# SKSKSK94/Distributed_SAC

Measured on AMD Instinct MI355X. Metric: learner grad-steps/sec (aggregate over GPUs), MT10-MTSAC, higher is better.
Workload: dtype bf16; 1 GPU; global_batch=1280, seq_len=1, parallelism=dp1, batch_per_gpu=1280, update=full SAC step: TD target + critic/actor/alpha fwd+bwd+fusedAdam + Polyak, hipgraph=True, launch_mode=graph, graph_chunk=1

## Files before the change

distributed_sac_amd/algo/sac.py:

```python

from __future__ import annotations

from typing import Dict, Optional

import torch
import torch.nn as nn

from ..config import SACConfig
from ..models import Actor, Critic, LLActor, LLCritic
from ..ops import functional as Fops
from ..ops.flat import FlatParams, FusedAdam, flat_polyak_


class SACEngine:

    def __init__(self, cfg: SACConfig, device: torch.device | str = "cpu",
                 precision: Optional[str] = None):
        import os as _os
        self.precision = (precision or
                          _os.environ.get("DSAC_PRECISION", "fp32"))
        self.cfg = cfg
        self.variant = cfg.variant
        self.device = torch.device(device)
        self.gamma = cfg.gamma
# ... 132 lines not shown
            device=self.device)
        off = self.actor_group.adopt_grad_arena(self._aa_arena, 0)
        self.alpha_group.adopt_grad_arena(self._aa_arena, off)
        self._init_bf16_mirrors()
        self.hard_copy_targets()

    def _init_bf16_mirrors(self) -> None:
        self._bf16 = (self.precision == "bf16"
                      and self.device.type == "cuda")
        if not self._bf16:
            return
        dev = self.device
        self._loss_ws = torch.zeros(256, device=dev)
        self._aloss_ws = torch.zeros(256, device=dev)
        self._dla_ws = torch.zeros(2048, device=dev)
        self._rng_ctr = torch.tensor(
            [int(torch.initial_seed()) & 0x7FFFFFFF],
            dtype=torch.int64, device=dev)
        self._critic_bf16 = torch.empty(self.critic_group.numel,
                                        dtype=torch.bfloat16, device=dev)
        self._target_bf16 = torch.empty(self.target_group.numel,
                                        dtype=torch.bfloat16, device=dev)
        self._actor_bf16 = torch.empty(self.actor_group.numel,
                                       dtype=torch.bfloat16, device=dev)
        self._twin_local_bf16 = self._stack_views(self.critic_group,
                                                  self._critic_bf16,
                                                  self._critic_layer_pairs())
        self._twin_target_bf16 = self._stack_views(
            self.target_group, self._target_bf16,
            self._critic_layer_pairs(target=True))
# ... 286 lines not shown
            self.ddp.allreduce_grad_(self._aa_arena)
        return self._manual_seg3()

    @property
    def _use_chain(self) -> bool:
        import os as _os
        return _os.environ.get("DSAC_CHAIN", "1") == "1"

    @property
    def _use_krng(self) -> bool:
        import os as _os
        return (getattr(self, "_bf16", False)
                and getattr(self, "_rng_ctr", None) is not None
                and _os.environ.get("DSAC_KRNG", "1") == "1")

    def _adam_prolog_all(self) -> bool:
        from ..ops import native
        opts = [self.critic_optimizer, self.actor_optimizer,
                self.log_alpha_optimizer]
        ctx = getattr(self, "context_encoder_optimizer", None)
        if ctx is not None:
            opts.append(ctx)
        if any(o._dev_state is None for o in opts):
            return False
        b1, b2 = opts[0].betas
        if any(o.betas != (b1, b2) or o.eps != opts[0].eps for o in opts):
            return False
        native().adam_prolog_many(
            [o._dev_state for o in opts], [o.lr for o in opts], b1, b2,
            self._rng_ctr if self._use_krng else None)
# ... 62 lines not shown
            mu, lsr, eps, float(self.actor.k),
            self._rng_ctr if krng else None)
        na, nlp = a_cat[:B], lp_cat[:B]

        if chain:
            yt, _ = self._chain_fwd(next_states, na,
                                    self._twin_target_bf16,
                                    self._twin_target[1], G=2,
                                    save_acts=False,
                                    wps=self._twin_target_fp)
            q1_t, q2_t = yt[0], yt[1]
        else:
            xt = torch.cat([next_states, na], dim=-1)
            q1_t, q2_t, _ = self._twin_fwd_manual(
                xt, self._twin_target_bf16, self._twin_target[1])
        y = ext.td_target_mt(rewards, dones, q1_t, q2_t, nlp, states,
                             la_det, T, self.gamma, self.reward_scale)

        if chain:
            yq, acts_c = self._chain_fwd(states, actions,
                                         self._twin_local_bf16,
                                         self._twin_local[1], G=2,
                                         wps=self._twin_local_fp)
            q1, q2 = yq[0], yq[1]
        else:
            x = torch.cat([states, actions], dim=-1)
            q1, q2, acts_c = self._twin_fwd_manual(
                x, self._twin_local_bf16, self._twin_local[1])
        closs = ext.critic_loss_fwd(q1, q2, y, states, la_det, T,
                                    int(use_w), self._loss_ws)[0]
        dy = ext.critic_loss_bwd2(q1, q2, y, states, la_det, closs, T,
                                  int(use_w))
        wsg = [w.grad for w in self._twin_local[0]]
        bsg = [b.grad for b in self._twin_local[1]]
        fg_c = self.critic_group.flat_grad
        arena_c, S_c, ch_c = self._dw_arena("critic",
                                            self.critic_group.numel, B)
        if chain:
            nl_c = len(self._twin_local_bf16)
            empty_h = states.new_empty(0, dtype=torch.bfloat16)
            youts = [acts_c[i + 1] for i in range(nl_c - 1)] + [empty_h]
            aflags = [1] * (nl_c - 1) + [0]
            dys = ext.mlp_chain_dx_bf16(dy, list(self._twin_local_wt),
                                        youts, acts_c[0].shape[-1],
                                        aflags, 2, 1, -1,
                                        list(self._twin_local_dxp))
            base_c = fg_c.data_ptr()
            ext.dwdb_grouped_arena(
                list(dys), [acts_c[i] for i in range(nl_c)], arena_c,
                [(w.data_ptr() - base_c) // 4 for w in wsg],
                [(b.data_ptr() - base_c) // 4 for b in bsg],
                2, S_c, ch_c)
        else:
            self._mlp_bwd_arena(ext, dy, acts_c, self._twin_local_bf16,
                                wsg, bsg, fg_c, arena_c, S_c, ch_c, G=2)
        ext.reduce_arena(arena_c, fg_c, S_c)
        self._dp_st = {
            "states": states, "sa": a_cat[B:], "lp": lp_cat[B:],
            "lsr": lsr, "ls_cat": ls_cat, "eps": eps, "tanh_u": tanh_u,
            "acts_a": acts_a, "ws_f32": ws_f32, "bs_f32": bs_f32,
            "la_det": la_det, "closs": closs, "B": B,
        }

    @torch.no_grad()
    def _manual_seg2(self):
        from ..ops import native
        ext = native()
        st = self._dp_st
        st["prolog"] = self._adam_prolog_all()
        self.critic_optimizer.step(pre_prologed=st["prolog"])

        states, sa, lp = st["states"], st["sa"], st["lp"]
        B = st["B"]
        T = self.num_tasks
        use_w = self.use_weighted_loss
        la_det = st["la_det"]
        ls = st["ls_cat"][B:]
        nl_a = len(self._actor_ws_bf16)
        nl_c = len(self._twin_local_bf16)
        acts_a = st["acts_a"]

        if self._use_chain:
            ext.pack_weights_frag(
                list(self._twin_local_bf16) * 2,
                list(self._twin_local_fp) + list(self._twin_local_dxp),
                [2] * (2 * nl_c), [0] * nl_c + [1] * nl_c)
            ya, acts_f = self._chain_fwd(states, sa, self._twin_local_bf16,
                                         self._twin_local[1], G=2,
                                         wps=self._twin_local_fp)
            aq1, aq2 = ya[0], ya[1]
        else:
            xa = torch.cat([states, sa], dim=-1)
            aq1, aq2, acts_f = self._twin_fwd_manual(
                xa, self._twin_local_bf16, self._twin_local[1])
        al = ext.actor_alpha_loss_fwd(aq1, aq2, lp, ls, states,
                                      la_det, T, int(use_w), self.H_bar_f,
                                      self.alpha_group.flat_grad,
                                      self._aloss_ws)
        daq, dlp = ext.actor_alpha_loss_bwd2(
            aq1, aq2, lp, states, la_det, al, self.alpha_group.flat_grad,
            T, int(use_w), self.H_bar_f, self._dla_ws)
        if self._use_chain:
            empty_h = states.new_empty(0, dtype=torch.bfloat16)
            youts_f = [acts_f[i + 1] for i in range(nl_c - 1)] + [empty_h]
            outs = ext.mlp_chain_dx_bf16(
                daq, list(self._twin_local_wt), youts_f,
                acts_f[0].shape[-1], [1] * (nl_c - 1) + [0], 2, 0,
                states.shape[1], list(self._twin_local_dxp))
            dx0 = outs[-1]
            dsa = dx0
        else:
            dy = daq
            for i in range(nl_c - 1, 0, -1):
                act = 1 if i < nl_c - 1 else 0
                yout = acts_f[i + 1] if i < nl_c - 1 else acts_f[i]
                dy = ext.linear_bwd_dx_bf16(dy, self._twin_local_bf16[i],
# ... 27 lines not shown
                [(b.data_ptr() - base_a) // 4 for b in bag],
                1, S_a, ch_a)
        else:
            dy = dhead
            for i in range(nl_a - 1, -1, -1):
                act = 1 if i < nl_a - 1 else 0
                yout = (acts_a[i + 1][B:] if i < nl_a - 1
                        else acts_a[i][B:])
                ext.linear_bwd_dwdb_arena(
                    dy, acts_a[i][B:], yout, act, 1, arena_a,
                    (wag[i].data_ptr() - base_a) // 4,
                    (bag[i].data_ptr() - base_a) // 4, S_a, ch_a, 0)
                if i > 0:
                    dy = ext.linear_bwd_dx_bf16(dy, self._actor_ws_bf16[i],
                                                yout, act, 1, 1)
        ext.reduce_arena(arena_a, fg_a, S_a)
        st["al"] = al

    @torch.no_grad()
    def _manual_seg3(self):
        st = self._dp_st
        FusedAdam.step_many([self.actor_optimizer,
                             self.log_alpha_optimizer],
                            rng_bump=(None if st.get("prolog")
                                      else (self._rng_ctr if self._use_krng
                                            else None)),
                            pre_prologed=bool(st.get("prolog")))
        flat_polyak_(self.target_group, self.critic_group, self.tau,
                     mirror=getattr(self, "_target_bf16", None))
        closs, al = st["closs"], st["al"]
        return {
            "critic_loss": closs[6],
            "actor_loss": al[0],
            "alpha_loss": al[2],
            "entropy": al[3],
        }

    def _update_tensors_fused(self, batch):
        from ..ops import native
        states = batch["states"]
        actions = batch["actions"]
        rewards = batch["rewards"]
        next_states = batch["next_states"]
        dones = batch["dones"]
# ... 192 lines not shown
```

distributed_sac_amd/ops/_hip/dsac_kernels.hip:

```cpp

#include <hip/hip_runtime.h>
#include <torch/extension.h>
#include <ATen/hip/HIPContext.h>
#include <c10/hip/HIPStream.h>

#include <cmath>
#include <vector>

using f32x4 = __attribute__((__vector_size__(4 * sizeof(float)))) float;

static constexpr int BM = 64;
static constexpr int BN = 64;
static constexpr int BK = 32;
static constexpr int PAD_K = BK + 2;
static constexpr int PAD_N = 80;

#define CHECK_IN(t) TORCH_CHECK((t).is_cuda() && (t).scalar_type() == torch::kFloat32, \
                                #t " must be a fp32 HIP tensor")

static inline hipStream_t cur_stream() {
  return c10::hip::getCurrentHIPStream().stream();
}

__global__ __launch_bounds__(256) void k_linear_act_fwd(
// ... 383 lines not shown
    const float mask = (raw >= -20.f && raw <= 2.f) ? 1.f : 0.f;
    dlsr[idx] = mask * (du * e * s - g);
  }
}

__global__ __launch_bounds__(256) void k_td_target(
    const float* __restrict__ r, const float* __restrict__ d,
    const float* __restrict__ q1, const float* __restrict__ q2,
    const float* __restrict__ lp, const float* __restrict__ alpha,
    float* __restrict__ y, int n, float gamma, float rs) {
  const int i = blockIdx.x * blockDim.x + threadIdx.x;
  if (i >= n) return;
  y[i] = rs * r[i] + gamma * (1.f - d[i]) * (fminf(q1[i], q2[i]) - alpha[i] * lp[i]);
}

__global__ __launch_bounds__(256) void k_td_target_mt(
    const float* __restrict__ r, const float* __restrict__ d,
    const float* __restrict__ q1, const float* __restrict__ q2,
    const float* __restrict__ lp, const float* __restrict__ onehot,
    const float* __restrict__ log_alpha, float* __restrict__ y,
    int n, int T, int oh_stride, float gamma, float rs) {
  const int i = blockIdx.x * blockDim.x + threadIdx.x;
  if (i >= n) return;
  int t_i = 0;
  if (T > 1) {
    float best = -1e30f;
    for (int t = 0; t < T; ++t) {
      const float v = onehot[(long)i * oh_stride + t];
      if (v > best) { best = v; t_i = t; }
    }
  }
  const float alpha = __expf(log_alpha[t_i]);
  y[i] = rs * r[i] + gamma * (1.f - d[i]) * (fminf(q1[i], q2[i]) - alpha * lp[i]);
}


__device__ __forceinline__ int task_of_row(const float* __restrict__ onehot,
                                           long i, int oh_stride, int T) {
  if (T <= 1) return 0;
  int t_i = 0;
  float best = -1e30f;
  for (int t = 0; t < T; ++t) {
    const float v = onehot[i * oh_stride + t];
    if (v > best) { best = v; t_i = t; }
  }
  return t_i;
}

// ... 556 lines not shown
  m[i] = mi;
  v[i] = vi;
  const float pn = p[i] - st[1] * mi / (sqrtf(vi) * st[2] + eps);
  p[i] = pn;
  if (mr != nullptr) mr[i] = f32_bf16_rne_d(pn);
}

__global__ __launch_bounds__(256) void k_polyak(
    float* __restrict__ t, const float* __restrict__ s, long n, float tau,
    unsigned short* __restrict__ mir) {
  const long i = (long)blockIdx.x * blockDim.x + threadIdx.x;
  if (i >= n) return;
  const float tn = (1.f - tau) * t[i] + tau * s[i];
  t[i] = tn;
  if (mir != nullptr) mir[i] = f32_bf16_rne_d(tn);
}


static torch::Tensor linear_act_fwd_g(torch::Tensor x, torch::Tensor w,
                                      torch::Tensor b, long act, long G) {
  CHECK_IN(x); CHECK_IN(w); CHECK_IN(b);
  auto xc = x.contiguous(); auto wc = w.contiguous(); auto bc = b.contiguous();
  const bool per_group_x = xc.dim() == 3;
  const long M = per_group_x ? xc.size(1) : xc.size(0);
  const long K = xc.size(-1);
  const long N = wc.numel() / (G * K);
  TORCH_CHECK(wc.numel() == G * N * K && bc.numel() == G * N,
              "grouped weight shape mismatch");
  const long xgs = per_group_x ? M * K : 0;
  auto y = G == 1 ? torch::empty({M, N}, xc.options())
// ... 382 lines not shown
    ws_p = ws->data_ptr<float>();
  }
  hipLaunchKernelGGL(k_actor_alpha_loss_bwd2,
                     dim3(ws_p ? nblk : nblk + 1),
                     dim3(256),
                     ws_p ? 0 : (size_t)T * 256 * sizeof(float),
                     cur_stream(), aq1.data_ptr<float>(),
                     aq2.data_ptr<float>(), lp.data_ptr<float>(), oh,
                     log_alpha.data_ptr<float>(), saved.data_ptr<float>(),
                     (unsigned short*)daq.data_ptr(), dlp.data_ptr<float>(),
                     dla_out.data_ptr<float>(), ws_p, (int)B, (int)T,
                     (int)oh_stride, (int)use_w, (float)H_bar);
  return {daq, dlp};
}

static torch::Tensor squashed_gaussian_bwd2(
    torch::Tensor ga, torch::Tensor gl, torch::Tensor lsr, torch::Tensor ls,
    torch::Tensor eps, torch::Tensor tanh_u, double k) {
  CHECK_IN(ga);
  auto gac = ga.contiguous(); auto glc = gl.contiguous();
  const bool lsr_ok = lsr.dim() == 2 && lsr.stride(1) == 1;
  auto lsrc = lsr_ok ? lsr : lsr.contiguous();
  auto lsc = ls.contiguous();
  auto ec = eps.contiguous(); auto tc = tanh_u.contiguous();
  const int ga_twin = (gac.dim() == 3 && gac.size(0) == 2) ? 1 : 0;
  const long B = ga_twin ? gac.size(1) : gac.size(0);
  const long A = ga_twin ? gac.size(2) : gac.size(1);
  const long lsr_ld = lsr_ok ? lsr.stride(0) : A;
  auto dhead = torch::empty({B, 2 * A},
                            gac.options().dtype(torch::kBFloat16));
// ... 15 lines not shown
  const double bc1 = 1.0 - std::pow(b1, (double)step);
  const double bc2 = 1.0 - std::pow(b2, (double)step);
  const float step_size = (float)(lr / bc1);
  const float inv_sqrt_bc2 = (float)(1.0 / std::sqrt(bc2));
  hipLaunchKernelGGL(k_adam, dim3((n + 255) / 256), dim3(256), 0,
                     cur_stream(), p.data_ptr<float>(), g.data_ptr<float>(),
                     m.data_ptr<float>(), v.data_ptr<float>(), n,
                     (float)b1, (float)b2, step_size, inv_sqrt_bc2,
                     (float)eps);
}

static void adam_step_dev_(torch::Tensor p, torch::Tensor g, torch::Tensor m,
                           torch::Tensor v, torch::Tensor state, double lr,
                           double b1, double b2, double eps,
                           c10::optional<torch::Tensor> mir_opt,
                           long skip_prolog = 0) {
  CHECK_IN(p); CHECK_IN(state);
  TORCH_CHECK(state.numel() >= 3, "state = {step, step_size, inv_sqrt_bc2}");
  const long n = p.numel();
  unsigned short* mp = nullptr;
  if (mir_opt.has_value() && mir_opt->defined() && mir_opt->numel() > 0) {
    TORCH_CHECK(mir_opt->numel() == n
                && mir_opt->scalar_type() == torch::kBFloat16);
    mp = (unsigned short*)mir_opt->data_ptr();
  }
  if (!skip_prolog)
    hipLaunchKernelGGL(k_adam_prolog, dim3(1), dim3(1), 0, cur_stream(),
                       state.data_ptr<float>(), (float)lr, (float)b1,
                       (float)b2);
  hipLaunchKernelGGL(k_adam_dev, dim3((n + 255) / 256), dim3(256), 0,
                     cur_stream(), p.data_ptr<float>(), g.data_ptr<float>(),
                     m.data_ptr<float>(), v.data_ptr<float>(),
                     state.data_ptr<float>(), n, (float)b1, (float)b2,
                     (float)eps, mp);
}

static void adam_prolog_many(std::vector<torch::Tensor> states,
                             std::vector<double> lrs, double b1, double b2,
                             c10::optional<torch::Tensor> rng) {
  const size_t G = states.size();
  TORCH_CHECK(G >= 1 && G <= 4 && lrs.size() == G, "1..4 states");
  float* S[4] = {nullptr, nullptr, nullptr, nullptr};
  double L[4] = {0, 0, 0, 0};
  for (size_t g = 0; g < G; ++g) {
// ... 5 lines not shown
      ? (long long*)rng->data_ptr<long>() : nullptr;
  hipLaunchKernelGGL(k_adam_prolog_many, dim3(1), dim3(4), 0, cur_stream(),
                     rng_p, S[0], S[1], S[2], S[3], (float)L[0],
                     (float)L[1], (float)L[2], (float)L[3], (float)b1,
                     (float)b2);
}

static void adam_step_multi_(std::vector<torch::Tensor> ps,
                             std::vector<torch::Tensor> gs,
                             std::vector<torch::Tensor> ms,
                             std::vector<torch::Tensor> vs,
                             std::vector<torch::Tensor> states,
                             std::vector<double> lrs, double b1, double b2,
                             double eps, std::vector<torch::Tensor> mirs,
                             c10::optional<torch::Tensor> rng = c10::nullopt,
                             long skip_prolog = 0) {
  const size_t G = ps.size();
  TORCH_CHECK(G >= 1 && G <= 3, "1..3 groups");
  float* P[3] = {nullptr, nullptr, nullptr};
  const float* Gr[3] = {nullptr, nullptr, nullptr};
  float* M[3] = {nullptr, nullptr, nullptr};
  float* V[3] = {nullptr, nullptr, nullptr};
  float* St[3] = {nullptr, nullptr, nullptr};
  long N[3] = {0, 0, 0};
  double LR[3] = {0, 0, 0};
  unsigned short* MR[3] = {nullptr, nullptr, nullptr};
  long total = 0;
  for (size_t g = 0; g < G; ++g) {
    CHECK_IN(ps[g]);
    P[g] = ps[g].data_ptr<float>();
    Gr[g] = gs[g].data_ptr<float>();
// ... 3 lines not shown
    N[g] = ps[g].numel();
    LR[g] = lrs[g];
    if (g < mirs.size() && mirs[g].defined() && mirs[g].numel() > 0) {
      TORCH_CHECK(mirs[g].numel() == N[g]
                  && mirs[g].scalar_type() == torch::kBFloat16);
      MR[g] = (unsigned short*)mirs[g].data_ptr();
    }
    total += N[g];
  }
  long long* rng_p = (rng.has_value() && rng->numel() > 0)
      ? (long long*)rng->data_ptr<long>() : nullptr;
  if (!skip_prolog)
    hipLaunchKernelGGL(k_adam_prolog3, dim3(1), dim3(3), 0, cur_stream(),
                       rng_p, St[0], St[1], St[2], (float)LR[0],
                       (float)LR[1], (float)LR[2], (float)b1, (float)b2);
  hipLaunchKernelGGL(k_adam_multi, dim3((total + 255) / 256), dim3(256), 0,
                     cur_stream(),
                     P[0], Gr[0], M[0], V[0], St[0], N[0],
                     P[1], Gr[1], M[1], V[1], St[1], N[1],
                     P[2], Gr[2], M[2], V[2], St[2], N[2],
                     (float)b1, (float)b2, (float)eps, MR[0], MR[1], MR[2]);
}

static void polyak_(torch::Tensor t, torch::Tensor s, double tau,
                    c10::optional<torch::Tensor> mir_opt) {
  CHECK_IN(t);
  const long n = t.numel();
  TORCH_CHECK(s.numel() == n, "polyak buffers must match");
  unsigned short* mp = nullptr;
  if (mir_opt.has_value() && mir_opt->defined() && mir_opt->numel() > 0) {
// ... 44 lines not shown
          pybind11::arg("aq1"), pybind11::arg("aq2"),
          pybind11::arg("lp"), pybind11::arg("ls"),
          pybind11::arg("states"), pybind11::arg("log_alpha"),
          pybind11::arg("T"), pybind11::arg("use_w"),
          pybind11::arg("H_bar"),
          pybind11::arg("dla") = pybind11::none(),
          pybind11::arg("ws") = pybind11::none());
  mod.def("actor_alpha_loss_bwd", &actor_alpha_loss_bwd);
  mod.def("critic_loss_bwd2", &critic_loss_bwd2);
  mod.def("actor_alpha_loss_bwd2", &actor_alpha_loss_bwd2,
          pybind11::arg("aq1"), pybind11::arg("aq2"), pybind11::arg("lp"),
          pybind11::arg("states"), pybind11::arg("log_alpha"),
          pybind11::arg("saved"), pybind11::arg("dla_out"),
          pybind11::arg("T"), pybind11::arg("use_w"), pybind11::arg("H_bar"),
          pybind11::arg("ws") = pybind11::none());
  mod.def("squashed_gaussian_bwd2", &squashed_gaussian_bwd2);
  mod.def("adam_step_", &adam_step_);
  mod.def("adam_step_dev_", &adam_step_dev_,
          pybind11::arg("p"), pybind11::arg("g"), pybind11::arg("m"),
          pybind11::arg("v"), pybind11::arg("state"), pybind11::arg("lr"),
          pybind11::arg("b1"), pybind11::arg("b2"), pybind11::arg("eps"),
          pybind11::arg("mir") = pybind11::none(),
          pybind11::arg("skip_prolog") = 0);
  mod.def("adam_step_multi_", &adam_step_multi_,
          pybind11::arg("ps"), pybind11::arg("gs"), pybind11::arg("ms"),
          pybind11::arg("vs"), pybind11::arg("states"), pybind11::arg("lrs"),
          pybind11::arg("b1"), pybind11::arg("b2"), pybind11::arg("eps"),
          pybind11::arg("mirs") = std::vector<torch::Tensor>(),
          pybind11::arg("rng") = pybind11::none(),
          pybind11::arg("skip_prolog") = 0);
  mod.def("adam_prolog_many", &adam_prolog_many,
          pybind11::arg("states"), pybind11::arg("lrs"),
          pybind11::arg("b1"), pybind11::arg("b2"),
          pybind11::arg("rng") = pybind11::none());
  mod.def("polyak_", &polyak_,
          pybind11::arg("t"), pybind11::arg("s"), pybind11::arg("tau"),
          pybind11::arg("mir") = pybind11::none());
}
```

distributed_sac_amd/ops/flat.py:

```python

from __future__ import annotations

import math
from typing import Dict, Iterable, List, Optional

import torch
import torch.nn as nn

from . import has_native, native, native_enabled


def _flatten_into(params: List[torch.Tensor]) -> torch.Tensor:
    numel = sum(p.numel() for p in params)
    if numel == 0:
        return torch.empty(0)
    flat = torch.empty(numel, dtype=torch.float32, device=params[0].device)
    off = 0
    for p in params:
        n = p.numel()
        flat[off:off + n].copy_(p.detach().reshape(-1))
        off += n
    return flat


# ... 86 lines not shown
        if self._dev_state is not None:
            return int(self._dev_state[0].item())
        return self._step_count

    @step_count.setter
    def step_count(self, v: int) -> None:
        self._step_count = int(v)
        if self._dev_state is not None:
            with torch.no_grad():
                self._dev_state[0] = float(v)

    def zero_grad(self) -> None:
        self.group.zero_grad()

    @torch.no_grad()
    def step(self, pre_prologed: bool = False) -> None:
        p, g = self.group.flat_data, self.group.flat_grad
        m, v = self.exp_avg, self.exp_avg_sq
        b1, b2 = self.betas
        if self._dev_state is not None:
            native().adam_step_dev_(p, g, m, v, self._dev_state,
                                    self.lr, b1, b2, self.eps,
                                    self.bf16_mirror,
                                    1 if pre_prologed else 0)
            return
        self._step_count += 1
        bc1 = 1 - b1 ** self._step_count
        bc2 = 1 - b2 ** self._step_count
        m.mul_(b1).add_(g, alpha=1 - b1)
        v.mul_(b2).addcmul_(g, g, value=1 - b2)
        denom = (v.sqrt() / math.sqrt(bc2)).add_(self.eps)
        p.addcdiv_(m, denom, value=-self.lr / bc1)

    @staticmethod
    @torch.no_grad()
    def step_many(opts: List["FusedAdam"], rng_bump=None,
                  pre_prologed: bool = False) -> None:
        live = [o for o in opts if o is not None]
        if (1 <= len(live) <= 3
                and all(o._dev_state is not None for o in live)
                and all(o.betas == live[0].betas and o.eps == live[0].eps
                        for o in live)):
            native().adam_step_multi_(
                [o.group.flat_data for o in live],
                [o.group.flat_grad for o in live],
                [o.exp_avg for o in live],
                [o.exp_avg_sq for o in live],
                [o._dev_state for o in live],
                [o.lr for o in live],
                live[0].betas[0], live[0].betas[1], live[0].eps,
                [o.bf16_mirror if o.bf16_mirror is not None
                 else torch.Tensor() for o in live],
                rng_bump, 1 if pre_prologed else 0)
            return
        for o in live:
            o.step()


    def state_dict(self) -> Dict:
        state = {}
        for i, (p, off) in enumerate(zip(self.ref_params, self._ref_offsets)):
            n = p.numel()
            state[i] = {
                "step": torch.tensor(float(self.step_count)),
                "exp_avg": self.exp_avg[off:off + n].view_as(p.data).clone(),
                "exp_avg_sq": self.exp_avg_sq[off:off + n].view_as(p.data).clone(),
            }
        group = {
            "lr": self.lr, "betas": self.betas, "eps": self.eps,
            "weight_decay": 0, "amsgrad": False, "maximize": False,
            "foreach": None, "capturable": False, "differentiable": False,
# ... 31 lines not shown
```

Before: 3244 grad_steps/s.

## Fuse SAC step tail: TD+critic loss, actor/alpha loss, arena reduce into Adam, Polyak

Merges the TD-target, critic loss forward and critic loss backward into one kernel, using a last-block-done atomic for the cross-block reduction. It also merges the actor/alpha loss forward and backward into one kernel. On single-GPU runs, the per-slice gradient-arena reduction is folded into the Adam step kernels and the Polyak target update is folded into the actor/alpha Adam launch. Together these cut several small kernel launches per step, at the cost of more complex kernels with grid-wide atomics and redundant per-block weight-sum scans.

Result: faster. 3444 grad_steps/s, median of 6 (+6.1%).

```diff
diff --git a/distributed_sac_amd/algo/sac.py b/distributed_sac_amd/algo/sac.py
--- a/distributed_sac_amd/algo/sac.py
+++ b/distributed_sac_amd/algo/sac.py
@@ -170,6 +170,7 @@
         self._loss_ws = torch.zeros(256, device=dev)
         self._aloss_ws = torch.zeros(256, device=dev)
         self._dla_ws = torch.zeros(2048, device=dev)
+        self._aafb_ws = torch.zeros(1 + 32 * 4 + 32 * 32, device=dev)
         self._rng_ctr = torch.tensor(
             [int(torch.initial_seed()) & 0x7FFFFFFF],
             dtype=torch.int64, device=dev)
@@ -486,6 +487,11 @@
                 and getattr(self, "_rng_ctr", None) is not None
                 and _os.environ.get("DSAC_KRNG", "1") == "1")
 
+    @property
+    def _fuse_tail(self) -> bool:
+        import os as _os
+        return _os.environ.get("DSAC_FUSE_TAIL", "1") == "1"
+
     def _adam_prolog_all(self) -> bool:
         from ..ops import native
         opts = [self.critic_optimizer, self.actor_optimizer,
@@ -578,8 +584,11 @@
             xt = torch.cat([next_states, na], dim=-1)
             q1_t, q2_t, _ = self._twin_fwd_manual(
                 xt, self._twin_target_bf16, self._twin_target[1])
-        y = ext.td_target_mt(rewards, dones, q1_t, q2_t, nlp, states,
-                             la_det, T, self.gamma, self.reward_scale)
+        fuse = self._fuse_tail
+        fuse_loss = fuse and B <= 8192
+        if not fuse_loss:
+            y = ext.td_target_mt(rewards, dones, q1_t, q2_t, nlp, states,
+                                 la_det, T, self.gamma, self.reward_scale)
 
         if chain:
             yq, acts_c = self._chain_fwd(states, actions,
@@ -591,10 +600,15 @@
             x = torch.cat([states, actions], dim=-1)
             q1, q2, acts_c = self._twin_fwd_manual(
                 x, self._twin_local_bf16, self._twin_local[1])
-        closs = ext.critic_loss_fwd(q1, q2, y, states, la_det, T,
-                                    int(use_w), self._loss_ws)[0]
-        dy = ext.critic_loss_bwd2(q1, q2, y, states, la_det, closs, T,
-                                  int(use_w))
+        if fuse_loss:
+            closs, dy = ext.critic_td_loss(
+                rewards, dones, q1_t, q2_t, nlp, q1, q2, states, la_det, T,
+                int(use_w), self.gamma, self.reward_scale, self._loss_ws)
+        else:
+            closs = ext.critic_loss_fwd(q1, q2, y, states, la_det, T,
+                                        int(use_w), self._loss_ws)[0]
+            dy = ext.critic_loss_bwd2(q1, q2, y, states, la_det, closs, T,
+                                      int(use_w))
         wsg = [w.grad for w in self._twin_local[0]]
         bsg = [b.grad for b in self._twin_local[1]]
         fg_c = self.critic_group.flat_grad
@@ -618,8 +632,11 @@
         else:
             self._mlp_bwd_arena(ext, dy, acts_c, self._twin_local_bf16,
                                 wsg, bsg, fg_c, arena_c, S_c, ch_c, G=2)
-        ext.reduce_arena(arena_c, fg_c, S_c)
+        fold_c = fuse and self.ddp is None
+        if not fold_c:
+            ext.reduce_arena(arena_c, fg_c, S_c)
         self._dp_st = {
+            "fuse": fuse, "arena_c": (arena_c, S_c) if fold_c else None,
             "states": states, "sa": a_cat[B:], "lp": lp_cat[B:],
             "lsr": lsr, "ls_cat": ls_cat, "eps": eps, "tanh_u": tanh_u,
             "acts_a": acts_a, "ws_f32": ws_f32, "bs_f32": bs_f32,
@@ -632,7 +649,8 @@
         ext = native()
         st = self._dp_st
         st["prolog"] = self._adam_prolog_all()
-        self.critic_optimizer.step(pre_prologed=st["prolog"])
+        self.critic_optimizer.step(pre_prologed=st["prolog"],
+                                   arena=st["arena_c"])
 
         states, sa, lp = st["states"], st["sa"], st["lp"]
         B = st["B"]
@@ -657,13 +675,22 @@
             xa = torch.cat([states, sa], dim=-1)
             aq1, aq2, acts_f = self._twin_fwd_manual(
                 xa, self._twin_local_bf16, self._twin_local[1])
-        al = ext.actor_alpha_loss_fwd(aq1, aq2, lp, ls, states,
-                                      la_det, T, int(use_w), self.H_bar_f,
-                                      self.alpha_group.flat_grad,
-                                      self._aloss_ws)
-        daq, dlp = ext.actor_alpha_loss_bwd2(
-            aq1, aq2, lp, states, la_det, al, self.alpha_group.flat_grad,
-            T, int(use_w), self.H_bar_f, self._dla_ws)
+        fuse = st["fuse"]
+        if fuse and B <= 8192:
+            al, daq, dlp = ext.actor_alpha_loss_fwd_bwd(
+                aq1, aq2, lp, ls, states, la_det,
+                self.alpha_group.flat_grad, T, int(use_w), self.H_bar_f,
+                self._aafb_ws, st["closs"][2:3] if use_w else None)
+        else:
+            al = ext.actor_alpha_loss_fwd(aq1, aq2, lp, ls, states,
+                                          la_det, T, int(use_w),
+                                          self.H_bar_f,
+                                          self.alpha_group.flat_grad,
+                                          self._aloss_ws)
+            daq, dlp = ext.actor_alpha_loss_bwd2(
+                aq1, aq2, lp, states, la_det, al,
+                self.alpha_group.flat_grad, T, int(use_w), self.H_bar_f,
+                self._dla_ws)
         if self._use_chain:
             empty_h = states.new_empty(0, dtype=torch.bfloat16)
             youts_f = [acts_f[i + 1] for i in range(nl_c - 1)] + [empty_h]
@@ -721,20 +748,28 @@
                 if i > 0:
                     dy = ext.linear_bwd_dx_bf16(dy, self._actor_ws_bf16[i],
                                                 yout, act, 1, 1)
-        ext.reduce_arena(arena_a, fg_a, S_a)
+        fold_a = fuse and self.ddp is None
+        if not fold_a:
+            ext.reduce_arena(arena_a, fg_a, S_a)
+        st["arena_a"] = (arena_a, S_a) if fold_a else None
         st["al"] = al
 
     @torch.no_grad()
     def _manual_seg3(self):
         st = self._dp_st
+        polyak = (self.target_group, self.critic_group, self.tau,
+                  getattr(self, "_target_bf16", None))
+        fuse = bool(st.get("fuse"))
         FusedAdam.step_many([self.actor_optimizer,
                              self.log_alpha_optimizer],
                             rng_bump=(None if st.get("prolog")
                                       else (self._rng_ctr if self._use_krng
                                             else None)),
-                            pre_prologed=bool(st.get("prolog")))
-        flat_polyak_(self.target_group, self.critic_group, self.tau,
-                     mirror=getattr(self, "_target_bf16", None))
+                            pre_prologed=bool(st.get("prolog")),
+                            arena0=st.get("arena_a"),
+                            polyak=polyak if fuse else None)
+        if not fuse:
+            flat_polyak_(*polyak)
         closs, al = st["closs"], st["al"]
         return {
             "critic_loss": closs[6],
diff --git a/distributed_sac_amd/ops/_hip/dsac_kernels.hip b/distributed_sac_amd/ops/_hip/dsac_kernels.hip
--- a/distributed_sac_amd/ops/_hip/dsac_kernels.hip
+++ b/distributed_sac_amd/ops/_hip/dsac_kernels.hip
@@ -421,6 +421,15 @@
   y[i] = rs * r[i] + gamma * (1.f - d[i]) * (fminf(q1[i], q2[i]) - alpha[i] * lp[i]);
 }
 
+__device__ __forceinline__ float td_target_value(float rs, float r,
+                                                 float gamma, float d,
+                                                 float qmin, float alpha,
+                                                 float lp) {
+#pragma clang fp contract(off)
+  const float x = __builtin_fmaf(-alpha, lp, qmin);
+  return rs * r + gamma * (1.f - d) * x;
+}
+
 __global__ __launch_bounds__(256) void k_td_target_mt(
     const float* __restrict__ r, const float* __restrict__ d,
     const float* __restrict__ q1, const float* __restrict__ q2,
@@ -438,7 +447,8 @@
     }
   }
   const float alpha = __expf(log_alpha[t_i]);
-  y[i] = rs * r[i] + gamma * (1.f - d[i]) * (fminf(q1[i], q2[i]) - alpha * lp[i]);
+  y[i] = td_target_value(rs, r[i], gamma, d[i], fminf(q1[i], q2[i]), alpha,
+                         lp[i]);
 }
 
 
@@ -1025,6 +1035,362 @@
   const float tn = (1.f - tau) * t[i] + tau * s[i];
   t[i] = tn;
   if (mir != nullptr) mir[i] = f32_bf16_rne_d(tn);
+}
+
+
+struct __attribute__((packed, aligned(4))) OneHot4 { float v[4]; };
+struct __attribute__((packed, aligned(4))) OneHot2 { float v[2]; };
+
+__device__ __forceinline__ float batch_weight_sum(
+    const float* __restrict__ smw, const float* __restrict__ onehot,
+    float (*wpart)[4], int B, int T, int oh_stride, int nblk, int& own_t) {
+  const int tid = threadIdx.x, wid = tid >> 6, lane = tid & 63;
+  constexpr int KR = 8;
+  for (int b0 = 0; b0 < nblk; b0 += KR) {
+    float best[KR];
+    int ti[KR];
+    long row[KR];
+#pragma unroll
+    for (int k = 0; k < KR; ++k) {
+      const int i = (b0 + k) * 256 + tid;
+      row[k] = (long)(i < B ? i : B - 1);
+      best[k] = -1e30f;
+      ti[k] = 0;
+    }
+    if (T > 1) {
+      int t = 0;
+#pragma unroll 2
+      for (; t + 4 <= T; t += 4) {
+#pragma unroll
+        for (int k = 0; k < KR; ++k) {
+          const OneHot4 q = *reinterpret_cast<const OneHot4*>(
+              onehot + row[k] * oh_stride + t);
+#pragma unroll
+          for (int c = 0; c < 4; ++c)
+            if (q.v[c] > best[k]) { best[k] = q.v[c]; ti[k] = t + c; }
+        }
+      }
+      if (t + 2 <= T) {
+#pragma unroll
+        for (int k = 0; k < KR; ++k) {
+          const OneHot2 q = *reinterpret_cast<const OneHot2*>(
+              onehot + row[k] * oh_stride + t);
+#pragma unroll
+          for (int c = 0; c < 2; ++c)
+            if (q.v[c] > best[k]) { best[k] = q.v[c]; ti[k] = t + c; }
+        }
+        t += 2;
+      }
+      if (t < T) {
+#pragma unroll
+        for (int k = 0; k < KR; ++k) {
+          const float v = onehot[row[k] * oh_stride + t];
+          if (v > best[k]) { best[k] = v; ti[k] = t; }
+        }
+      }
+    }
+    float w[KR];
+#pragma unroll
+    for (int k = 0; k < KR; ++k) {
+      const int i = (b0 + k) * 256 + tid;
+      w[k] = i < B ? smw[ti[k]] : 0.f;
+      if (b0 + k == (int)blockIdx.x) own_t = ti[k];
+    }
+#pragma unroll
+    for (int off = 32; off > 0; off >>= 1) {
+#pragma unroll
+      for (int k = 0; k < KR; ++k) w[k] += __shfl_xor(w[k], off, 64);
+    }
+#pragma unroll
+    for (int k = 0; k < KR; ++k)
+      if (lane == 0 && b0 + k < nblk) wpart[b0 + k][wid] = w[k];
+  }
+  __syncthreads();
+  float r = 0.f;
+  for (int b = 0; b < nblk; ++b)
+    r += wpart[b][0] + wpart[b][1] + wpart[b][2] + wpart[b][3];
+  return r;
+}
+
+__global__ __launch_bounds__(256) void k_critic_td_loss(
+    const float* __restrict__ r, const float* __restrict__ d,
+    const float* __restrict__ q1t, const float* __restrict__ q2t,
+    const float* __restrict__ nlp, const float* __restrict__ q1,
+    const float* __restrict__ q2, const float* __restrict__ onehot,
+    const float* __restrict__ log_alpha, float* __restrict__ out,
+    float* __restrict__ ws, unsigned short* __restrict__ dq,
+    int B, int T, int oh_stride, int use_w, float gamma, float rs) {
+  __shared__ float part[3][4];
+  __shared__ float smw[32];
+  __shared__ float wpart[32][4];
+  __shared__ float s_fin[32 * 3];
+  __shared__ int s_last;
+  const int tid = threadIdx.x;
+  const int i = blockIdx.x * 256 + tid;
+  const long ic = i < B ? i : B - 1;
+  const float rv = r[ic], dv = d[ic], q1tv = q1t[ic], q2tv = q2t[ic];
+  const float lpv = nlp[ic], q1v = q1[ic], q2v = q2[ic];
+  int t_i = 0;
+  float wsum = 1.f;
+  if (use_w) {
+    fill_task_weights(smw, log_alpha, T);
+    __syncthreads();
+    wsum = batch_weight_sum(smw, onehot, wpart, B, T, oh_stride,
+                            (int)gridDim.x, t_i);
+  } else {
+    t_i = task_of_row(onehot, ic, oh_stride, T);
+  }
+  float s_l1 = 0.f, s_l2 = 0.f, s_w = 0.f;
+  if (i < B) {
+    const float alpha = __expf(log_alpha[t_i]);
+    const float y = td_target_value(rs, rv, gamma, dv, fminf(q1tv, q2tv),
+                                    alpha, lpv);
+    const float w_raw = use_w ? smw[t_i] : 1.f;
+    s_w += w_raw;
+    const float d1 = y - q1v, d2 = y - q2v;
+    s_l1 += w_raw * d1 * d1;
+    s_l2 += w_raw * d2 * d2;
+    const float coeff = (use_w ? w_raw / wsum : 1.f) / (float)B;
+    dq[i] = f32_bf16_rne_d(coeff * -2.f * (y - q1v));
+    dq[B + i] = f32_bf16_rne_d(coeff * -2.f * (y - q2v));
+  }
+  s_l1 = wave_sum64(s_l1); s_l2 = wave_sum64(s_l2); s_w = wave_sum64(s_w);
+  const int wid = tid >> 6;
+  if ((tid & 63) == 0) {
+    part[0][wid] = s_l1; part[1][wid] = s_l2; part[2][wid] = s_w;
+  }
+  __syncthreads();
+  float* slots = ws + 1;
+  if (tid == 0) {
+    slots[blockIdx.x * 3 + 0] =
+        part[0][0] + part[0][1] + part[0][2] + part[0][3];
+    slots[blockIdx.x * 3 + 1] =
+        part[1][0] + part[1][1] + part[1][2] + part[1][3];
+    slots[blockIdx.x * 3 + 2] =
+        part[2][0] + part[2][1] + part[2][2] + part[2][3];
+    __threadfence();
+    const unsigned old = atomicAdd((unsigned*)ws, 1u);
+    s_last = (old == (unsigned)gridDim.x - 1u);
+    if (s_last) {
+      *(unsigned*)ws = 0u;
+      __threadfence();
+    }
+  }
+  __syncthreads();
+  if (!s_last) return;
+  const int nb = (int)gridDim.x;
+  if (tid < nb * 3) s_fin[tid] = ((const volatile float*)slots)[tid];
+  __syncthreads();
+  if (tid == 0) {
+    float r0 = 0.f, r1 = 0.f, r2 = 0.f;
+    for (int b = 0; b < nb; ++b) {
+      r0 += s_fin[b * 3 + 0];
+      r1 += s_fin[b * 3 + 1];
+      r2 += s_fin[b * 3 + 2];
+    }
+    const float wfin = use_w ? r2 : 1.f;
+    const float denom = wfin * (float)B;
+    out[3] = r0; out[4] = r1; out[5] = r2;
+    out[0] = r0 / denom;
+    out[1] = r1 / denom;
+    out[2] = wfin;
+    out[6] = (r0 + r1) / denom;
+  }
+}
+
+__global__ __launch_bounds__(256) void k_actor_alpha_loss_fwd_bwd(
+    const float* __restrict__ aq1, const float* __restrict__ aq2,
+    const float* __restrict__ lp, const float* __restrict__ ls,
+    const float* __restrict__ onehot, const float* __restrict__ log_alpha,
+    float* __restrict__ out, float* __restrict__ ws,
+    unsigned short* __restrict__ daq, float* __restrict__ dlp,
+    float* __restrict__ dla, int dla_n, const float* __restrict__ wsum_in,
+    int B, int T, int A, int oh_stride, int use_w, float H_bar) {
+  __shared__ float part[4][4];
+  __shared__ float smw[32];
+  __shared__ float wpart[32][4];
+  __shared__ float s_val[256];
+  __shared__ int s_t[256];
+  __shared__ int s_last;
+  __shared__ float s_fin[32 * 4];
+  __shared__ float s_g[32 * 32];
+  const int tid = threadIdx.x;
+  constexpr float CE = 1.4189385332046727f;
+  const int i = blockIdx.x * 256 + tid;
+  const long ic = i < B ? i : B - 1;
+  const float aq1v = aq1[ic], aq2v = aq2[ic], lpv = lp[ic];
+  float ent = CE * A;
+  for (int a = 0; a < A; ++a) ent += ls[ic * A + a];
+  int t_i = 0;
+  float wsum = 1.f;
+  if (use_w) {
+    fill_task_weights(smw, log_alpha, T);
+    __syncthreads();
+  }
+  if (use_w && wsum_in == nullptr) {
+    wsum = batch_weight_sum(smw, onehot, wpart, B, T, oh_stride,
+                            (int)gridDim.x, t_i);
+  } else {
+    if (use_w) wsum = wsum_in[0];
+    t_i = task_of_row(onehot, ic, oh_stride, T);
+  }
+  float s_pl = 0.f, s_w = 0.f, s_al = 0.f, s_en = 0.f;
+  s_t[tid] = -1;
+  s_val[tid] = 0.f;
+  if (i < B) {
+    s_t[tid] = t_i;
+    s_val[tid] = -(lpv + H_bar) / (float)B;
+    const float la = log_alpha[t_i];
+    const float alpha_i = __expf(la);
+    const float w_raw = use_w ? smw[t_i] : 1.f;
+    s_w += w_raw;
+    const float qmin = fminf(aq1v, aq2v);
+    s_pl += w_raw * -(qmin - alpha_i * lpv);
+    s_al += la * (lpv + H_bar);
+    s_en += ent;
+    const float coeff = (use_w ? w_raw / wsum : 1.f) / (float)B;
+    const bool first = aq1v <= aq2v;
+    daq[i] = f32_bf16_rne_d(first ? coeff * -1.f : 0.f);
+    daq[B + i] = f32_bf16_rne_d(first ? 0.f : coeff * -1.f);
+    dlp[i] = coeff * alpha_i;
+  }
+  s_pl = wave_sum64(s_pl); s_w = wave_sum64(s_w);
+  s_al = wave_sum64(s_al); s_en = wave_sum64(s_en);
+  const int wid = tid >> 6, lane = tid & 63;
+  if (lane == 0) {
+    part[0][wid] = s_pl; part[1][wid] = s_w;
+    part[2][wid] = s_al; part[3][wid] = s_en;
+  }
+  __syncthreads();
+  float* mslots = ws + 1;
+  float* gslots = ws + 1 + 32 * 4;
+  for (int t0 = wid; t0 < T; t0 += 16) {
+    float v[4];
+#pragma unroll
+    for (int j = 0; j < 4; ++j) {
+      const int t = t0 + 4 * j;
+      v[j] = ((s_t[lane] == t ? s_val[lane] : 0.f) +
+              (s_t[lane + 64] == t ? s_val[lane + 64] : 0.f)) +
+             ((s_t[lane + 128] == t ? s_val[lane + 128] : 0.f) +
+              (s_t[lane + 192] == t ? s_val[lane + 192] : 0.f));
+    }
+#pragma unroll
+    for (int off = 32; off > 0; off >>= 1) {
+#pragma unroll
+      for (int j = 0; j < 4; ++j) v[j] += __shfl_xor(v[j], off, 64);
+    }
+    if (lane == 0) {
+#pragma unroll
+      for (int j = 0; j < 4; ++j)
+        if (t0 + 4 * j < T) gslots[(long)blockIdx.x * T + t0 + 4 * j] = v[j];
+      __threadfence();
+    }
+  }
+  __syncthreads();
+  if (tid == 0) {
+#pragma unroll
+    for (int k = 0; k < 4; ++k)
+      mslots[blockIdx.x * 4 + k] =
+          part[k][0] + part[k][1] + part[k][2] + part[k][3];
+    __threadfence();
+    const unsigned old = atomicAdd((unsigned*)ws, 1u);
+    s_last = (old == (unsigned)gridDim.x - 1u);
+    if (s_last) { *(unsigned*)ws = 0u; __threadfence(); }
+  }
+  __syncthreads();
+  if (!s_last) return;
+  const int nb = (int)gridDim.x;
+  if (tid < nb * 4) s_fin[tid] = ((const volatile float*)mslots)[tid];
+  for (int k = tid; k < nb * T; k += 256)
+    s_g[k] = ((const volatile float*)gslots)[k];
+  __syncthreads();
+  if (tid < dla_n) {
+    float g = 0.f;
+    if (tid < T) {
+      float rsum = 0.f;
+      for (int b = 0; b < nb; ++b) rsum += s_g[b * T + tid];
+      g = 0.f + rsum;
+    }
+    dla[tid] = g;
+  }
+  if (tid == 0) {
+    float r0 = 0.f, r1 = 0.f, r2 = 0.f, r3 = 0.f;
+    for (int b = 0; b < nb; ++b) {
+      r0 += s_fin[b * 4 + 0]; r1 += s_fin[b * 4 + 1];
+      r2 += s_fin[b * 4 + 2]; r3 += s_fin[b * 4 + 3];
+    }
+    const float wfin = use_w ? r1 : 1.f;
+    out[4] = r0; out[5] = r1; out[6] = r2; out[7] = r3;
+    out[0] = r0 / (wfin * (float)B);
+    out[1] = wfin;
+    out[2] = -r2 / (float)B;
+    out[3] = r3 / (float)B;
+  }
+}
+
+__global__ __launch_bounds__(256) void k_adam_dev_arena(
+    float* __restrict__ p, float* __restrict__ g,
+    float* __restrict__ m, float* __restrict__ v,
+    const float* __restrict__ state, long n, float b1, float b2, float eps,
+    unsigned short* __restrict__ mir, const float* __restrict__ arena,
+    long stride, int S) {
+  const long i = (long)blockIdx.x * blockDim.x + threadIdx.x;
+  if (i >= n) return;
+  const float step_size = state[1], inv_sqrt_bc2 = state[2];
+  float acc = 0.f;
+  for (int s = 0; s < S; ++s) acc += arena[(long)s * stride + i];
+  g[i] = acc;
+  const float gi = acc;
+  const float mi = b1 * m[i] + (1.f - b1) * gi;
+  const float vi = b2 * v[i] + (1.f - b2) * gi * gi;
+  m[i] = mi;
+  v[i] = vi;
+  const float pn = p[i] - step_size * mi / (sqrtf(vi) * inv_sqrt_bc2 + eps);
+  p[i] = pn;
+  if (mir != nullptr) mir[i] = f32_bf16_rne_d(pn);
+}
+
+__global__ __launch_bounds__(256) void k_adam_multi_tail(
+    float* p0, float* g0, float* m0, float* v0, const float* st0, long n0,
+    float* p1, const float* g1, float* m1, float* v1, const float* st1, long n1,
+    float* p2, const float* g2, float* m2, float* v2, const float* st2, long n2,
+    float b1, float b2, float eps, unsigned short* mr0, unsigned short* mr1,
+    unsigned short* mr2, const float* __restrict__ arena0, long stride0,
+    int S0, float* __restrict__ pt, const float* __restrict__ psrc, long np,
+    float tau, unsigned short* __restrict__ pmir) {
+  long i = (long)blockIdx.x * blockDim.x + threadIdx.x;
+  float* p; const float* g; float* m; float* v; const float* st;
+  unsigned short* mr;
+  bool fold = false;
+  if (i < n0) {
+    p = p0; g = g0; m = m0; v = v0; st = st0; mr = mr0;
+    fold = arena0 != nullptr;
+  }
+  else if ((i -= n0) < n1) { p = p1; g = g1; m = m1; v = v1; st = st1; mr = mr1; }
+  else if ((i -= n1) < n2) { p = p2; g = g2; m = m2; v = v2; st = st2; mr = mr2; }
+  else if ((i -= n2) < np) {
+    const float tn = (1.f - tau) * pt[i] + tau * psrc[i];
+    pt[i] = tn;
+    if (pmir != nullptr) pmir[i] = f32_bf16_rne_d(tn);
+    return;
+  }
+  else return;
+  float gi;
+  if (fold) {
+    float acc = 0.f;
+    for (int s = 0; s < S0; ++s) acc += arena0[(long)s * stride0 + i];
+    g0[i] = acc;
+    gi = acc;
+  } else {
+    gi = g[i];
+  }
+  const float mi = b1 * m[i] + (1.f - b1) * gi;
+  const float vi = b2 * v[i] + (1.f - b2) * gi * gi;
+  m[i] = mi;
+  v[i] = vi;
+  const float pn = p[i] - st[1] * mi / (sqrtf(vi) * st[2] + eps);
+  p[i] = pn;
+  if (mr != nullptr) mr[i] = f32_bf16_rne_d(pn);
 }
 
 
@@ -1437,6 +1803,89 @@
   return {daq, dlp};
 }
 
+static std::vector<torch::Tensor> critic_td_loss(
+    torch::Tensor r, torch::Tensor d, torch::Tensor q1t, torch::Tensor q2t,
+    torch::Tensor nlp, torch::Tensor q1, torch::Tensor q2,
+    torch::Tensor states, torch::Tensor log_alpha, long T, long use_w,
+    double gamma, double rs, torch::Tensor ws) {
+  CHECK_IN(r); CHECK_IN(d); CHECK_IN(q1t); CHECK_IN(q2t); CHECK_IN(nlp);
+  CHECK_IN(q1); CHECK_IN(q2); CHECK_IN(states); CHECK_IN(log_alpha);
+  CHECK_IN(ws);
+  const long B = q1.size(0);
+  const long nblk = (B + 255) / 256;
+  TORCH_CHECK(B >= 1 && nblk <= 32, "critic_td_loss: 1 <= B <= 8192");
+  TORCH_CHECK(T >= 1 && T <= 32 && log_alpha.numel() >= T, "T <= 32");
+  TORCH_CHECK(ws.numel() >= 1 + 32 * 3, "workspace too small");
+  TORCH_CHECK(states.dim() == 2 && states.is_contiguous()
+              && states.size(0) == B && states.size(1) >= T);
+  auto rc = r.contiguous(); auto dc = d.contiguous();
+  auto q1tc = q1t.contiguous(); auto q2tc = q2t.contiguous();
+  auto lpc = nlp.contiguous();
+  auto q1c = q1.contiguous(); auto q2c = q2.contiguous();
+  TORCH_CHECK(rc.numel() == B && dc.numel() == B && q1tc.numel() == B
+              && q2tc.numel() == B && lpc.numel() == B && q1c.numel() == B
+              && q2c.numel() == B, "critic_td_loss: B elements per input");
+  const long oh_stride = states.size(1);
+  const float* oh = states.data_ptr<float>() + (oh_stride - T);
+  auto out = torch::empty({8}, q1.options());
+  auto dq = torch::empty({2, B, 1}, q1.options().dtype(torch::kBFloat16));
+  hipLaunchKernelGGL(k_critic_td_loss, dim3(nblk), dim3(256), 0,
+                     cur_stream(), rc.data_ptr<float>(),
+                     dc.data_ptr<float>(), q1tc.data_ptr<float>(),
+                     q2tc.data_ptr<float>(), lpc.data_ptr<float>(),
+                     q1c.data_ptr<float>(), q2c.data_ptr<float>(), oh,
+                     log_alpha.data_ptr<float>(), out.data_ptr<float>(),
+                     ws.data_ptr<float>(), (unsigned short*)dq.data_ptr(),
+                     (int)B, (int)T, (int)oh_stride, (int)use_w,
+                     (float)gamma, (float)rs);
+  return {out, dq};
+}
+
+static std::vector<torch::Tensor> actor_alpha_loss_fwd_bwd(
+    torch::Tensor aq1, torch::Tensor aq2, torch::Tensor lp, torch::Tensor ls,
+    torch::Tensor states, torch::Tensor log_alpha, torch::Tensor dla,
+    long T, long use_w, double H_bar, torch::Tensor ws,
+    c10::optional<torch::Tensor> wsum = c10::nullopt) {
+  CHECK_IN(aq1); CHECK_IN(aq2); CHECK_IN(lp); CHECK_IN(ls);
+  CHECK_IN(states); CHECK_IN(log_alpha); CHECK_IN(dla); CHECK_IN(ws);
+  const float* wsum_p = nullptr;
+  if (wsum.has_value() && wsum->defined() && wsum->numel() > 0) {
+    CHECK_IN(*wsum);
+    wsum_p = wsum->data_ptr<float>();
+  }
+  const long B = aq1.size(0);
+  const long nblk = (B + 255) / 256;
+  TORCH_CHECK(B >= 1 && nblk <= 32,
+              "actor_alpha_loss_fwd_bwd: 1 <= B <= 8192");
+  TORCH_CHECK(T >= 1 && T <= 32 && log_alpha.numel() >= T
+              && dla.numel() >= T && dla.numel() <= 256
+              && dla.is_contiguous(), "alpha gradient: T <= 32");
+  TORCH_CHECK(ws.numel() >= 1 + 32 * 4 + nblk * T, "workspace too small");
+  TORCH_CHECK(states.dim() == 2 && states.is_contiguous()
+              && states.size(0) == B && states.size(1) >= T);
+  auto aq1c = aq1.contiguous(); auto aq2c = aq2.contiguous();
+  auto lpc = lp.contiguous(); auto lsc = ls.contiguous();
+  TORCH_CHECK(aq1c.numel() == B && aq2c.numel() == B && lpc.numel() == B
+              && lsc.dim() == 2 && lsc.size(0) == B,
+              "actor_alpha_loss_fwd_bwd: B rows per input");
+  const long A = lsc.size(1);
+  const long oh_stride = states.size(1);
+  const float* oh = states.data_ptr<float>() + (oh_stride - T);
+  auto out = torch::empty({8}, aq1.options());
+  auto daq = torch::empty({2, B, 1}, aq1.options().dtype(torch::kBFloat16));
+  auto dlp = torch::empty_like(lpc);
+  hipLaunchKernelGGL(k_actor_alpha_loss_fwd_bwd, dim3(nblk), dim3(256), 0,
+                     cur_stream(), aq1c.data_ptr<float>(),
+                     aq2c.data_ptr<float>(), lpc.data_ptr<float>(),
+                     lsc.data_ptr<float>(), oh, log_alpha.data_ptr<float>(),
+                     out.data_ptr<float>(), ws.data_ptr<float>(),
+                     (unsigned short*)daq.data_ptr(), dlp.data_ptr<float>(),
+                     dla.data_ptr<float>(), (int)dla.numel(), wsum_p, (int)B,
+                     (int)T, (int)A, (int)oh_stride, (int)use_w,
+                     (float)H_bar);
+  return {out, daq, dlp};
+}
+
 static torch::Tensor squashed_gaussian_bwd2(
     torch::Tensor ga, torch::Tensor gl, torch::Tensor lsr, torch::Tensor ls,
     torch::Tensor eps, torch::Tensor tanh_u, double k) {
@@ -1482,10 +1931,21 @@
                            torch::Tensor v, torch::Tensor state, double lr,
                            double b1, double b2, double eps,
                            c10::optional<torch::Tensor> mir_opt,
-                           long skip_prolog = 0) {
+                           long skip_prolog = 0,
+                           c10::optional<torch::Tensor> arena = c10::nullopt,
+                           long S = 0) {
   CHECK_IN(p); CHECK_IN(state);
   TORCH_CHECK(state.numel() >= 3, "state = {step, step_size, inv_sqrt_bc2}");
   const long n = p.numel();
+  const float* ap = nullptr;
+  if (arena.has_value() && arena->defined() && arena->numel() > 0) {
+    CHECK_IN(*arena); CHECK_IN(g);
+    TORCH_CHECK(arena->dim() == 2 && arena->is_contiguous()
+                && g.is_contiguous() && arena->size(1) == n
+                && g.numel() == n && S >= 1 && S <= arena->size(0),
+                "arena must be [>=S, numel]");
+    ap = arena->data_ptr<float>();
+  }
   unsigned short* mp = nullptr;
   if (mir_opt.has_value() && mir_opt->defined() && mir_opt->numel() > 0) {
     TORCH_CHECK(mir_opt->numel() == n
@@ -1496,6 +1956,14 @@
     hipLaunchKernelGGL(k_adam_prolog, dim3(1), dim3(1), 0, cur_stream(),
                        state.data_ptr<float>(), (float)lr, (float)b1,
                        (float)b2);
+  if (ap != nullptr) {
+    hipLaunchKernelGGL(k_adam_dev_arena, dim3((n + 255) / 256), dim3(256), 0,
+                       cur_stream(), p.data_ptr<float>(),
+                       g.data_ptr<float>(), m.data_ptr<float>(),
+                       v.data_ptr<float>(), state.data_ptr<float>(), n,
+                       (float)b1, (float)b2, (float)eps, mp, ap, n, (int)S);
+    return;
+  }
   hipLaunchKernelGGL(k_adam_dev, dim3((n + 255) / 256), dim3(256), 0,
                      cur_stream(), p.data_ptr<float>(), g.data_ptr<float>(),
                      m.data_ptr<float>(), v.data_ptr<float>(),
@@ -1531,7 +1999,13 @@
                              std::vector<double> lrs, double b1, double b2,
                              double eps, std::vector<torch::Tensor> mirs,
                              c10::optional<torch::Tensor> rng = c10::nullopt,
-                             long skip_prolog = 0) {
+                             long skip_prolog = 0,
+                             c10::optional<torch::Tensor> arena0 = c10::nullopt,
+                             long S0 = 0,
+                             c10::optional<torch::Tensor> polyak_t = c10::nullopt,
+                             c10::optional<torch::Tensor> polyak_s = c10::nullopt,
+                             double tau = 0.0,
+                             c10::optional<torch::Tensor> polyak_mir = c10::nullopt) {
   const size_t G = ps.size();
   TORCH_CHECK(G >= 1 && G <= 3, "1..3 groups");
   float* P[3] = {nullptr, nullptr, nullptr};
@@ -1565,6 +2039,46 @@
     hipLaunchKernelGGL(k_adam_prolog3, dim3(1), dim3(3), 0, cur_stream(),
                        rng_p, St[0], St[1], St[2], (float)LR[0],
                        (float)LR[1], (float)LR[2], (float)b1, (float)b2);
+  const float* ap = nullptr;
+  if (arena0.has_value() && arena0->defined() && arena0->numel() > 0) {
+    CHECK_IN(*arena0); CHECK_IN(gs[0]);
+    TORCH_CHECK(arena0->dim() == 2 && arena0->is_contiguous()
+                && gs[0].is_contiguous() && arena0->size(1) == N[0]
+                && gs[0].numel() == N[0] && S0 >= 1
+                && S0 <= arena0->size(0), "arena0 must be [>=S0, numel0]");
+    ap = arena0->data_ptr<float>();
+  }
+  float* pt = nullptr; const float* psrc = nullptr; long np = 0;
+  unsigned short* pmir = nullptr;
+  if (polyak_t.has_value() && polyak_t->defined() && polyak_t->numel() > 0) {
+    TORCH_CHECK(polyak_s.has_value(), "polyak source missing");
+    CHECK_IN(*polyak_t); CHECK_IN(*polyak_s);
+    np = polyak_t->numel();
+    TORCH_CHECK(polyak_s->numel() == np && polyak_t->is_contiguous()
+                && polyak_s->is_contiguous(), "polyak buffers must match");
+    for (size_t g = 0; g < G; ++g)
+      TORCH_CHECK(polyak_s->data_ptr() != ps[g].data_ptr()
+                  && polyak_t->data_ptr() != ps[g].data_ptr(),
+                  "polyak buffers must not be stepped in the same launch");
+    pt = polyak_t->data_ptr<float>();
+    psrc = polyak_s->data_ptr<float>();
+    if (polyak_mir.has_value() && polyak_mir->defined()
+        && polyak_mir->numel() > 0) {
+      TORCH_CHECK(polyak_mir->numel() == np
+                  && polyak_mir->scalar_type() == torch::kBFloat16);
+      pmir = (unsigned short*)polyak_mir->data_ptr();
+    }
+  }
+  if (ap != nullptr || pt != nullptr) {
+    hipLaunchKernelGGL(k_adam_multi_tail, dim3((total + np + 255) / 256),
+                       dim3(256), 0, cur_stream(),
+                       P[0], gs[0].data_ptr<float>(), M[0], V[0], St[0], N[0],
+                       P[1], Gr[1], M[1], V[1], St[1], N[1],
+                       P[2], Gr[2], M[2], V[2], St[2], N[2],
+                       (float)b1, (float)b2, (float)eps, MR[0], MR[1], MR[2],
+                       ap, N[0], (int)S0, pt, psrc, np, (float)tau, pmir);
+    return;
+  }
   hipLaunchKernelGGL(k_adam_multi, dim3((total + 255) / 256), dim3(256), 0,
                      cur_stream(),
                      P[0], Gr[0], M[0], V[0], St[0], N[0],
@@ -1639,6 +2153,19 @@
           pybind11::arg("saved"), pybind11::arg("dla_out"),
           pybind11::arg("T"), pybind11::arg("use_w"), pybind11::arg("H_bar"),
           pybind11::arg("ws") = pybind11::none());
+  mod.def("critic_td_loss", &critic_td_loss,
+          pybind11::arg("r"), pybind11::arg("d"), pybind11::arg("q1t"),
+          pybind11::arg("q2t"), pybind11::arg("nlp"), pybind11::arg("q1"),
+          pybind11::arg("q2"), pybind11::arg("states"),
+          pybind11::arg("log_alpha"), pybind11::arg("T"),
+          pybind11::arg("use_w"), pybind11::arg("gamma"),
+          pybind11::arg("rs"), pybind11::arg("ws"));
+  mod.def("actor_alpha_loss_fwd_bwd", &actor_alpha_loss_fwd_bwd,
+          pybind11::arg("aq1"), pybind11::arg("aq2"), pybind11::arg("lp"),
+          pybind11::arg("ls"), pybind11::arg("states"),
+          pybind11::arg("log_alpha"), pybind11::arg("dla"),
+          pybind11::arg("T"), pybind11::arg("use_w"), pybind11::arg("H_bar"),
+          pybind11::arg("ws"), pybind11::arg("wsum") = pybind11::none());
   mod.def("squashed_gaussian_bwd2", &squashed_gaussian_bwd2);
   mod.def("adam_step_", &adam_step_);
   mod.def("adam_step_dev_", &adam_step_dev_,
@@ -1646,14 +2173,22 @@
           pybind11::arg("v"), pybind11::arg("state"), pybind11::arg("lr"),
           pybind11::arg("b1"), pybind11::arg("b2"), pybind11::arg("eps"),
           pybind11::arg("mir") = pybind11::none(),
-          pybind11::arg("skip_prolog") = 0);
+          pybind11::arg("skip_prolog") = 0,
+          pybind11::arg("arena") = pybind11::none(),
+          pybind11::arg("S") = 0);
   mod.def("adam_step_multi_", &adam_step_multi_,
           pybind11::arg("ps"), pybind11::arg("gs"), pybind11::arg("ms"),
           pybind11::arg("vs"), pybind11::arg("states"), pybind11::arg("lrs"),
           pybind11::arg("b1"), pybind11::arg("b2"), pybind11::arg("eps"),
           pybind11::arg("mirs") = std::vector<torch::Tensor>(),
           pybind11::arg("rng") = pybind11::none(),
-          pybind11::arg("skip_prolog") = 0);
+          pybind11::arg("skip_prolog") = 0,
+          pybind11::arg("arena0") = pybind11::none(),
+          pybind11::arg("S0") = 0,
+          pybind11::arg("polyak_t") = pybind11::none(),
+          pybind11::arg("polyak_s") = pybind11::none(),
+          pybind11::arg("tau") = 0.0,
+          pybind11::arg("polyak_mir") = pybind11::none());
   mod.def("adam_prolog_many", &adam_prolog_many,
           pybind11::arg("states"), pybind11::arg("lrs"),
           pybind11::arg("b1"), pybind11::arg("b2"),
diff --git a/distributed_sac_amd/ops/flat.py b/distributed_sac_amd/ops/flat.py
--- a/distributed_sac_amd/ops/flat.py
+++ b/distributed_sac_amd/ops/flat.py
@@ -124,16 +124,27 @@
         self.group.zero_grad()
 
     @torch.no_grad()
-    def step(self, pre_prologed: bool = False) -> None:
+    def step(self, pre_prologed: bool = False, arena=None) -> None:
         p, g = self.group.flat_data, self.group.flat_grad
         m, v = self.exp_avg, self.exp_avg_sq
         b1, b2 = self.betas
         if self._dev_state is not None:
+            if arena is not None:
+                native().adam_step_dev_(p, g, m, v, self._dev_state,
+                                        self.lr, b1, b2, self.eps,
+                                        self.bf16_mirror,
+                                        1 if pre_prologed else 0,
+                                        arena[0], int(arena[1]))
+                return
             native().adam_step_dev_(p, g, m, v, self._dev_state,
                                     self.lr, b1, b2, self.eps,
                                     self.bf16_mirror,
                                     1 if pre_prologed else 0)
             return
+        if arena is not None:
+            g.zero_()
+            for s in range(int(arena[1])):
+                g.add_(arena[0][s])
         self._step_count += 1
         bc1 = 1 - b1 ** self._step_count
         bc2 = 1 - b2 ** self._step_count
@@ -145,13 +156,16 @@
     @staticmethod
     @torch.no_grad()
     def step_many(opts: List["FusedAdam"], rng_bump=None,
-                  pre_prologed: bool = False) -> None:
+                  pre_prologed: bool = False, arena0=None,
+                  polyak=None) -> None:
         live = [o for o in opts if o is not None]
+        assert arena0 is None or (opts and opts[0] is not None), \
+            "arena0 belongs to the first optimizer"
         if (1 <= len(live) <= 3
                 and all(o._dev_state is not None for o in live)
                 and all(o.betas == live[0].betas and o.eps == live[0].eps
                         for o in live)):
-            native().adam_step_multi_(
+            args = [
                 [o.group.flat_data for o in live],
                 [o.group.flat_grad for o in live],
                 [o.exp_avg for o in live],
@@ -161,10 +175,24 @@
                 live[0].betas[0], live[0].betas[1], live[0].eps,
                 [o.bf16_mirror if o.bf16_mirror is not None
                  else torch.Tensor() for o in live],
-                rng_bump, 1 if pre_prologed else 0)
+                rng_bump, 1 if pre_prologed else 0]
+            if arena0 is not None or polyak is not None:
+                args += [arena0[0] if arena0 is not None else None,
+                         int(arena0[1]) if arena0 is not None else 0]
+                if polyak is not None:
+                    target, source, tau, mirror = polyak
+                    assert target.numel == source.numel
+                    args += [target.flat_data, source.flat_data, float(tau),
+                             mirror]
+            native().adam_step_multi_(*args)
             return
-        for o in live:
-            o.step()
+        if rng_bump is not None and not pre_prologed:
+            rng_bump.add_(1)
+        for j, o in enumerate(live):
+            o.step(pre_prologed=pre_prologed,
+                   arena=arena0 if (j == 0 and o is opts[0]) else None)
+        if polyak is not None:
+            flat_polyak_(*polyak)
 
 
     def state_dict(self) -> Dict:
```
